# hongsukchoi/Pose2Mesh_RELEASE

Measured on NVIDIA H100. Metric: SMPL meshes/sec, higher is better.
Workload: dtype f32 (wgmma fp16x3 split, fp32 accumulate)

## Files before the change

pose2mesh_release_b200/csrc/cheb_umma.cu:

```cuda
#include <cuda.h>
#include <cuda_fp16.h>
#include <cuda_runtime.h>

#include <algorithm>
#include <climits>
#include <cstdlib>
#include <cstring>
#include <vector>

#include "p2m_internal.h"

namespace p2m {

namespace {

constexpr int TILE_M = 128;
constexpr int FC = 32;
constexpr int A_BLOCK_BYTES = TILE_M * 128;
constexpr float W_SCALE = 64.f;
constexpr float W_INV_SCALE = 1.f / 64.f;

struct TileHeader {
  int n_rows;
  int h1;
// ... 164 lines not shown
    fma4(acc0, __uint_as_float(a0.y), x0);
    fma4(acc1, __uint_as_float(a1.y), x1);
    fma4(acc0, __uint_as_float(a2.y), x2);
    fma4(acc1, __uint_as_float(a3.y), x3);
  }
  if (e + 1 < e1) {
    const uint2 a0 = lds_u2(ent + e * 8), a1 = lds_u2(ent + e * 8 + 8);
    const float4 x0 = lds_f4(rows_q + a0.x), x1 = lds_f4(rows_q + a1.x);
    fma4(acc0, __uint_as_float(a0.y), x0);
    fma4(acc1, __uint_as_float(a1.y), x1);
    e += 2;
  }
  if (e < e1) {
    const uint2 a0 = lds_u2(ent + e * 8);
    fma4(acc0, __uint_as_float(a0.y), lds_f4(rows_q + a0.x));
  }
  return make_float4(acc0.x + acc1.x, acc0.y + acc1.y, acc0.z + acc1.z, acc0.w + acc1.w);
}

__device__ __forceinline__ void wg_fence() { asm volatile("wgmma.fence.sync.aligned;" ::: "memory"); }
__device__ __forceinline__ void wg_commit() { asm volatile("wgmma.commit_group.sync.aligned;" ::: "memory"); }
__device__ __forceinline__ void wg_wait0() { asm volatile("wgmma.wait_group.sync.aligned 0;" ::: "memory"); }
template <int TA, int TB>
__device__ __forceinline__ void wgmma_m64n64(float (&d)[32], uint64_t desc_a, uint64_t desc_b) {
  asm volatile(
      "{\n\t.reg .pred p;\n\tsetp.ne.b32 p, 1, 0;\n\t"
      "wgmma.mma_async.sync.aligned.m64n64k16.f32.f16.f16 "
      "{%0, %1, %2, %3, %4, %5, %6, %7, %8, %9, %10, %11, %12, %13, %14, %15, "
      "%16, %17, %18, %19, %20, %21, %22, %23, %24, %25, %26, %27, %28, %29, %30, %31}, %32, %33, p, 1, 1, %34, %35;\n\t}"
      : "+f"(d[0]), "+f"(d[1]), "+f"(d[2]), "+f"(d[3]), "+f"(d[4]), "+f"(d[5]), "+f"(d[6]), "+f"(d[7]), "+f"(d[8]),
        "+f"(d[9]), "+f"(d[10]), "+f"(d[11]), "+f"(d[12]), "+f"(d[13]), "+f"(d[14]), "+f"(d[15]), "+f"(d[16]),
        "+f"(d[17]), "+f"(d[18]), "+f"(d[19]), "+f"(d[20]), "+f"(d[21]), "+f"(d[22]), "+f"(d[23]), "+f"(d[24]),
        "+f"(d[25]), "+f"(d[26]), "+f"(d[27]), "+f"(d[28]), "+f"(d[29]), "+f"(d[30]), "+f"(d[31])
      : "l"(desc_a), "l"(desc_b), "n"(TA), "n"(TB)
      : "memory");
}
template <int TA, int TB>
__device__ __forceinline__ void wgmma_m64n32(float (&d)[16], uint64_t desc_a, uint64_t desc_b) {
  asm volatile(
      "{\n\t.reg .pred p;\n\tsetp.ne.b32 p, 1, 0;\n\t"
      "wgmma.mma_async.sync.aligned.m64n32k16.f32.f16.f16 "
      "{%0, %1, %2, %3, %4, %5, %6, %7, %8, %9, %10, %11, %12, %13, %14, %15}, %16, %17, p, 1, 1, %18, %19;\n\t}"
      : "+f"(d[0]), "+f"(d[1]), "+f"(d[2]), "+f"(d[3]), "+f"(d[4]), "+f"(d[5]), "+f"(d[6]), "+f"(d[7]), "+f"(d[8]),
        "+f"(d[9]), "+f"(d[10]), "+f"(d[11]), "+f"(d[12]), "+f"(d[13]), "+f"(d[14]), "+f"(d[15])
      : "l"(desc_a), "l"(desc_b), "n"(TA), "n"(TB)
      : "memory");
}

__device__ __forceinline__ uint64_t make_desc_sw128(uint32_t saddr) {
  uint64_t d = 0;
  d |= (uint64_t)((saddr & 0x3FFFF) >> 4);
  d |= (uint64_t)1 << 16;
  d |= (uint64_t)(1024 >> 4) << 32;
  d |= (uint64_t)1 << 62;
  return d;
}

__host__ __device__ __forceinline__ uint32_t sw128_off(int row, int chunk) {
  return (uint32_t)row * 128u + (uint32_t)((chunk ^ (row & 7)) << 4);
}

struct Half4 {
  __half2 a, b;
};
__device__ __forceinline__ void split4(const float4& v, uint2& hi, uint2& lo) {
  __half2 h0 = __floats2half2_rn(v.x, v.y), h1 = __floats2half2_rn(v.z, v.w);
// ... 18 lines not shown
  EpiDev ep;
  int res_identity;
  const float* t1;
  const float* a_scale;
  const float* b_scale;
  long long ldy;
  int y_col0;
  float* y;
  int* status;
  long long* trace;
  int own_table;
  const float* head_wt;
  float* head_z;
  const unsigned char* apack;
  long long wslice_bytes;
  long long wblock_stride;
  int tma;
  CUtensorMap tm_x, tm_t1;
};

#ifdef P2M_UMMA_TRACE
__device__ __forceinline__ void trace_ev(const KParams& p, int role, int& n, int ev) {
  if (p.trace != nullptr && blockIdx.x == 0 && blockIdx.y == 0 && n < 512) {
    p.trace[role * 512 + n] = ((long long)ev << 48) | (clock64() & 0xFFFFFFFFFFFFll);
    ++n;
  }
}
#else
__device__ __forceinline__ void trace_ev(const KParams&, int, int&, int) {}
#endif

constexpr int W_PROD = 16;
constexpr int W_XLOAD = 16, N_XLOAD = 2, W_BLOAD = 18, W_EPI0 = 20;
constexpr int W_EPI1 = 8, W_PARK = 12;
constexpr int NUM_THREADS2 = 24 * 32;
constexpr int REGS_LAUNCH = 80, REGS_UTIL = 40, REGS_EPI = 120;
constexpr int REGS_PROD2 = 88, REGS_PARK = 24;
static_assert(128 * (REGS_EPI - REGS_LAUNCH) <= 128 * (REGS_LAUNCH - REGS_UTIL), "register pool balance");
static_assert(2 * 128 * (REGS_PROD2 - REGS_LAUNCH) + 2 * 128 * (REGS_EPI - REGS_LAUNCH) <=
                  128 * (REGS_LAUNCH - REGS_PARK) + 128 * (REGS_LAUNCH - REGS_UTIL),
              "register pool balance of the N = 128 layout");
static_assert(W_XLOAD % 4 == 0 && W_EPI0 % 4 == 0 && W_EPI0 - W_XLOAD == 4, "setmaxnreg works on aligned warpgroups");
static_assert(W_EPI1 % 4 == 0 && W_PARK == W_EPI1 + 4 && W_XLOAD == W_PARK + 4, "setmaxnreg works on aligned warpgroups");
template <int N>
__host__ __device__ constexpr int prod_warps() { return N == 128 ? W_EPI1 : W_PROD; }

template <int N>
__host__ __device__ constexpr int tile_rows() { return N == 128 ? 64 : TILE_M; }
template <int N, int NS, int XS, int MODE>
__global__ void __launch_bounds__(NUM_THREADS2, 1) k_cheb_conv_umma(const __grid_constant__ KParams p) {
  static_assert(N == 64 || N == 128, "one warpgroup holds the CTA's 128 x 64 or 64 x 128 accumulator in registers");
  constexpr int TM = tile_rows<N>();
  constexpr int NPW = prod_warps<N>();
  constexpr int NRG = NPW * 4;
  constexpr int RPT = TM / NRG;
  constexpr int NWG = N == 128 ? 2 : 1;
  static_assert(RPT == 2, "both configurations give a producer thread two tile rows");
  constexpr int H = TM / 64;
  constexpr int ER = 16 * H;
  constexpr bool KT1 = (MODE == 1);
  constexpr bool plain = !KT1;
  constexpr bool XDIRECT = KT1 && NS >= 3;
  constexpr int A_BYTES = TM * 128;
  constexpr int B_BLOCK_BYTES = N * 128;
  constexpr int SLOT_BYTES = A_BYTES + B_BLOCK_BYTES;

  extern __shared__ __align__(1024) unsigned char smem_raw[];
  unsigned char* ring = smem_raw;
  float* Xs = reinterpret_cast<float*>(ring + NS * SLOT_BYTES);
  const size_t xs_stage_floats = (XDIRECT && TM == 64) ? 0 : (size_t)TM * FC;
  float* T1s = Xs + XS * xs_stage_floats;
  const size_t t1_stage_floats = (size_t)p.max_h1 * FC;
  unsigned char* meta_s =
      reinterpret_cast<unsigned char*>(T1s + (plain ? 0 : XS) * t1_stage_floats);
  uint64_t* bars = reinterpret_cast<uint64_t*>(meta_s + 2 * (size_t)p.meta_stride);
  uint64_t* b_ab_full = bars;
  uint64_t* b_ab_empty = b_ab_full + NS;
  uint64_t* b_x_full = b_ab_empty + NS;
  uint64_t* b_x_empty = b_x_full + XS;
  uint64_t* b_m_full = b_x_empty + XS;
  uint64_t* b_m_empty = b_m_full + 2;
  uint64_t* b_stg_free = b_m_empty + 2;
  uint64_t* b_turn = b_stg_free + 1;
  uint32_t* flags = reinterpret_cast<uint32_t*>(b_turn + 1);
  volatile int* abort_flag = reinterpret_cast<volatile int*>(flags + 1);
  float* ep_mul = reinterpret_cast<float*>(flags + 4);
// ... 7 lines not shown
  uint64_t* b_res = reinterpret_cast<uint64_t*>(head_w_s);

  const int tid = threadIdx.x;
  const int warp = tid >> 5;
  const int lane = tid & 31;
  const int n_chunk = p.fin / FC;
  const int n_use = 3 * n_chunk;

  if (tid == 0) {
    for (int s = 0; s < NS; ++s) {
      mbar_init(smem_u32(b_ab_full + s), p.apack != nullptr ? 1 : NPW + 1);
      mbar_init(smem_u32(b_ab_empty + s), 4);
    }
    for (int s = 0; s < XS; ++s) {
      mbar_init(smem_u32(b_x_full + s), N_XLOAD * 32 + 1);
      mbar_init(smem_u32(b_x_empty + s), 1);
    }
    for (int s = 0; s < 2; ++s) {
      mbar_init(smem_u32(b_m_full + s), 1);
      mbar_init(smem_u32(b_m_empty + s), 1);
    }
    if (N == 128) {
      for (int w = 0; w < 4; ++w) mbar_init(smem_u32(b_res + w), 1);
      mbar_init(smem_u32(b_stg_free), 4);
      mbar_init(smem_u32(b_turn), 4);
    }
    *abort_flag = (smem_u32(ring) & 1023u) ? 1 : 0;
    if (*abort_flag) mbar_timeout(abort_flag, p.status, 100);
    fence_barrier_init();
  }
  const float a_scale = p.a_scale ? *p.a_scale : 1.f;
  const float b_inv = p.b_scale ? 1.f / *p.b_scale : W_INV_SCALE;
  const int ecol0 = (int)blockIdx.y * N;
  for (int n = threadIdx.x; n < N; n += NUM_THREADS2) {
    const float sc = (p.ep.scale ? p.ep.scale[ecol0 + n] : 1.f) / a_scale;
    const float sh = p.ep.scale ? p.ep.shift[ecol0 + n] : 0.f;
    const float bi = p.ep.bias ? p.ep.bias[ecol0 + n] : 0.f;
    ep_mul[n] = b_inv * sc;
    ep_add[n] = fmaf(bi, p.ep.scale ? p.ep.scale[ecol0 + n] : 1.f, sh);
  }
  if (N == 64 && p.head_z != nullptr)
    for (int i = threadIdx.x; i < 64 * 12; i += NUM_THREADS2) head_w_s[i] = p.head_wt[i];
  __syncthreads();

  const int mma_g = warp >= W_EPI0 ? 0 : (NWG == 2 && warp >= W_EPI1 && warp < W_PARK) ? 1 : -1;
  if (warp >= W_XLOAD && warp < W_EPI0) {
  asm volatile("setmaxnreg.dec.sync.aligned.u32 %0;" ::"n"(REGS_UTIL));
  if (warp >= W_XLOAD && warp < W_XLOAD + N_XLOAD) {
    if (p.apack == nullptr) {
      const int lt = tid - W_XLOAD * 32;
      const int lq = lt & 7, lrg = lt >> 3;
      const int my_tiles = (p.n_tiles - (int)blockIdx.x + (int)gridDim.x - 1) / (int)gridDim.x;
      if (lt == 32 && p.tma) {
        if (!XDIRECT) asm volatile("prefetch.tensormap [%0];" ::"l"(reinterpret_cast<uint64_t>(&p.tm_x)) : "memory");
        if (KT1) asm volatile("prefetch.tensormap [%0];" ::"l"(reinterpret_cast<uint64_t>(&p.tm_t1)) : "memory");
      }
      auto fetch_meta = [&](int itf) {
        const int pat = (blockIdx.x + itf * gridDim.x) % p.P;
        const int m = itf & 1;
        mbar_wait_relaxed(smem_u32(b_m_empty + m), ((itf >> 1) & 1) ^ 1, abort_flag, p.status, 1);
        const int mbytes = p.meta_bytes[pat];
        mbar_arrive_expect_tx(smem_u32(b_m_full + m), mbytes);
        bulk_g2s(smem_u32(meta_s + (size_t)m * p.meta_stride), p.meta + (size_t)pat * p.meta_stride, mbytes,
                 smem_u32(b_m_full + m));
      };
      if (lt == 0 && my_tiles > 0) fetch_meta(0);
      const uint32_t fin_bytes = (uint32_t)p.fin * 4u;
      const int sh = p.in_unpool ? 1 : 0;
      int g2 = 0;
      int ltn = 0;
      for (int it2 = 0; it2 < my_tiles; ++it2) {
        const int tile2 = blockIdx.x + it2 * gridDim.x;
        const long long mesh_row0 = (long long)(tile2 / p.P) * p.V;
        const int m2 = it2 & 1;
        mbar_wait_relaxed(smem_u32(b_m_full + m2), (it2 >> 1) & 1, abort_flag, p.status, 8);
        const unsigned char* mb2 = meta_s + (size_t)m2 * p.meta_stride;
        const TileHeader* hdr2 = reinterpret_cast<const TileHeader*>(mb2);
        const int* halo = reinterpret_cast<const int*>(mb2 + hdr2->off_halo);
        const int h1 = hdr2->h1;
        for (int c2 = 0; c2 < n_chunk; ++c2, ++g2) {
          const int xs2 = g2 % XS;
          mbar_wait_relaxed(smem_u32(b_x_empty + xs2), ((g2 / XS) & 1) ^ 1, abort_flag, p.status, 11);
          if (lt == 0) trace_ev(p, 4, ltn, 1);
// ... 8 lines not shown
                if (v[u] != -2) {
                  const uint32_t srow = (uint32_t)max(v[u], 0) >> shift;
                  cp_async16_zfill(dbase + (i0 + 8 * u) * 128, sbase + (uint64_t)srow * (uint64_t)fin_bytes,
                                   v[u] >= 0 ? 16u : 0u);
                }
              }
            }
          };
          const char* t1_mesh =
              reinterpret_cast<const char*>(KT1 ? p.t1 + mesh_row0 * p.fin + c2 * FC + lq * 4 : nullptr);
          const char* x_mesh = reinterpret_cast<const char*>(p.x + (mesh_row0 >> sh) * p.fin + c2 * FC + lq * 4);
          const uint32_t t1_dst = smem_u32(T1s + xs2 * t1_stage_floats) + lq * 16;
          const uint32_t x_dst = smem_u32(Xs + xs2 * xs_stage_floats) + lq * 16;
          if (p.tma) {
            if (lt == 32) {
              const int own0 = tile2 * TM;
              mbar_arrive_expect_tx(xbar, (XDIRECT ? 0 : (p.in_unpool ? TM / 2 : TM) * 128) + (KT1 ? TM * 128 : 0));
              if (!XDIRECT)
                tma_load_2d(smem_u32(Xs + xs2 * xs_stage_floats), &p.tm_x, c2 * FC, p.in_unpool ? own0 >> 1 : own0, xbar);
              if (KT1) tma_load_2d(smem_u32(T1s + xs2 * t1_stage_floats), &p.tm_t1, c2 * FC, own0, xbar);
            }
            if (KT1) stage_rows(t1_dst, t1_mesh, TM, h1, 0);
          } else {
            if (KT1) stage_rows(t1_dst, t1_mesh, 0, h1, 0);
            if (!XDIRECT) stage_rows(x_dst, x_mesh, 0, TM, sh);
            if (lt == 32) mbar_arrive(xbar);
          }
          cp_async_arrive_noinc(xbar);
          if (lt == 0) trace_ev(p, 4, ltn, 2);
          if (lt == 0 && c2 == (n_chunk > 1 ? 1 : 0) && it2 + 1 < my_tiles) fetch_meta(it2 + 1);
        }
      }
    }
  } else if (warp == W_BLOAD) {
    if (lane == 0) {
      uint32_t ucnt = 0;
      int tn = 0;
      const int uses = plain ? n_chunk : n_use;
      for (int tile = blockIdx.x; tile < p.n_tiles; tile += gridDim.x) {
        for (int u = 0; u < uses; ++u, ++ucnt) {
          const int s = ucnt % NS;
          const uint32_t par = (ucnt / NS) & 1;
          mbar_wait_relaxed(smem_u32(b_ab_empty + s), par ^ 1, abort_flag, p.status, 4);
          trace_ev(p, 1, tn, 10 + u);
          const unsigned char* wsl = p.wpack + (size_t)blockIdx.y * (size_t)p.wslice_bytes;
          if (p.apack != nullptr) {
            mbar_arrive_expect_tx(smem_u32(b_ab_full + s), B_BLOCK_BYTES + A_BYTES);
            bulk_g2s(smem_u32(ring + s * SLOT_BYTES), p.apack + ((size_t)tile * uses + u) * A_BYTES, A_BYTES,
                     smem_u32(b_ab_full + s));
          } else {
            mbar_arrive_expect_tx(smem_u32(b_ab_full + s), B_BLOCK_BYTES);
          }
          bulk_g2s(smem_u32(ring + s * SLOT_BYTES + A_BYTES), wsl + (size_t)u * (size_t)p.wblock_stride, B_BLOCK_BYTES,
                   smem_u32(b_ab_full + s));
        }
      }
    }
  }
  } else if (mma_g >= 0) {
    asm volatile("setmaxnreg.inc.sync.aligned.u32 %0;" ::"n"(REGS_EPI));
    const int g = mma_g;
    const int wq = warp - (g == 0 ? W_EPI0 : W_EPI1);
    const int tr = 3 + 2 * g;
    constexpr int CPR = EC / 4;
    constexpr int RPI = 32 / CPR;
    const uint32_t stg = smem_u32(epi_stage) + (uint32_t)wq * STG_WARP_BYTES;
    const int prow = lane / CPR, pc = lane % CPR;
    constexpr int NP = ER / RPI;
    int colk[2];
#pragma unroll
    for (int k = 0; k < 2; ++k) colk[k] = (int)(((uint32_t)pc ^ (uint32_t)((k * RPI + prow) & 7)) << 2);
    const int trow = (lane >> 4) * 64 + wq * 16 + (lane & 15);
    const int uses = plain ? n_chunk : n_use;
    int etn = 0;
    for (int it = g; (int)blockIdx.x + it * (int)gridDim.x < p.n_tiles; it += NWG) {
      const int tile = blockIdx.x + it * gridDim.x;
      const int b = tile / p.P, pat = tile - b * p.P;
      const long long mesh0 = (long long)b * p.V;
      int* own_w = own_s + (g * 4 + wq) * ER;
      {
        int v;
        if (lane >= ER) {
          v = -1;
        } else if (p.own_table) {
          v = __ldg(reinterpret_cast<const int*>(p.meta + (size_t)pat * p.meta_stride + 64) + trow);
        } else {
          v = pat * TM + trow;
          if (v >= p.V) v = -1;
        }
        __syncwarp();
        if (lane < ER) own_w[lane] = v;
        __syncwarp();
      }
      int own_v[NP];
#pragma unroll
      for (int i = 0; i < NP; ++i) own_v[i] = own_w[i * RPI + prow];
      if (p.ep.res != nullptr) {
        const bool own_cols = p.apack != nullptr || (N == 128 && p.res_identity);
        const int lpr = ((own_cols ? N : p.ep.res_F) * 4 + 127) >> 7;
        for (int j = lane; j < ER * lpr; j += 32) {
          const int rr = j / lpr, ln = j - rr * lpr;
          const int vtx = own_w[rr];
          if (vtx >= 0) {
            const long long r = mesh0 + vtx;
            prefetch_l2(p.ep.res + (p.ep.res_unpool ? (r >> 1) : r) * p.ep.res_F + (own_cols ? ecol0 : 0) + ln * 32);
          }
        }
      }
      float acc[2][32];
#pragma unroll
      for (int h = 0; h < 2; ++h)
#pragma unroll
        for (int j = 0; j < 32; ++j) acc[h][j] = 0.f;
      if (wq == 0 && lane == 0) trace_ev(p, tr, etn, 1);
      if (NWG == 2 && it > 0) {
        mbar_wait(smem_u32(b_turn), (uint32_t)(it - 1) & 1u, abort_flag, p.status, 13);
        if (wq == 0 && lane == 0) trace_ev(p, tr, etn, 3);
      }
      uint32_t ucnt = (uint32_t)it * (uint32_t)uses;
      for (int u = 0; u < uses; ++u, ++ucnt) {
        const uint32_t s = ucnt % NS;
        if (wq == 0 && lane == 0) trace_ev(p, tr, etn, 4);
        mbar_wait(smem_u32(b_ab_full + s), (ucnt / NS) & 1, abort_flag, p.status, 6);
        if (wq == 0 && lane == 0) trace_ev(p, tr, etn, 5);
        const uint32_t a0 = smem_u32(ring + s * SLOT_BYTES);
        wg_fence();
#pragma unroll
        for (int h = 0; h < 2; ++h) {
          const uint64_t da = make_desc_sw128(a0 + (TM == 128 ? (uint32_t)h * (64 * 128) : 0u));
          const uint64_t db = make_desc_sw128(a0 + A_BYTES + (TM == 64 ? (uint32_t)h * (64 * 128) : 0u));
          wgmma_m64n64<0, 0>(acc[h], da + 0, db + 0);
          wgmma_m64n64<0, 0>(acc[h], da + 2, db + 2);
          wgmma_m64n64<0, 0>(acc[h], da + 4, db + 0);
          wgmma_m64n64<0, 0>(acc[h], da + 6, db + 2);
          wgmma_m64n64<0, 0>(acc[h], da + 0, db + 4);
          wgmma_m64n64<0, 0>(acc[h], da + 2, db + 6);
        }
        wg_commit();
        wg_wait0();
        __syncwarp();
        if (lane == 0) mbar_arrive(smem_u32(b_ab_empty + s));
      }
      if (NWG == 2 && lane == 0) mbar_arrive(smem_u32(b_turn));
      if (wq == 0 && lane == 0) trace_ev(p, tr, etn, 2);
      auto stage_slab = [&](int cb) {
#pragma unroll
        for (int h = 0; h < H; ++h)
#pragma unroll
          for (int jj = 0; jj < 4; ++jj)
#pragma unroll
            for (int r = 0; r < 2; ++r) {
              const int lr = 16 * h + (lane >> 2) + 8 * r;
              const int cc = 8 * jj + 2 * (lane & 3);
              const int j = 4 * (cb / 8 + jj) + 2 * r;
              sts_f2(stg + lr * (EC * 4) + ((((uint32_t)(cc >> 2)) ^ (uint32_t)(lr & 7)) << 4) + (cc & 3) * 4,
                     acc[h][j], acc[h][j + 1]);
            }
        __syncwarp();
      };
      if (N == 64 && p.head_z != nullptr) {
        float z[12];
#pragma unroll
        for (int j = 0; j < 12; ++j) z[j] = 0.f;
#pragma unroll
        for (int cb = 0; cb < N; cb += 32) {
          stage_slab(cb);
#pragma unroll
          for (int c = 0; c < 8; ++c) {
            const float4 a = lds_f4(stg + lane * (EC * 4) + (((uint32_t)c ^ (uint32_t)(lane & 7)) << 4));
// ... 109 lines not shown
            const int n = cb + colk[i & 1];
            const int gn = ecol0 + n;
            const float4 a = lds_f4(stg + rr * (EC * 4) + (pc << 4));
            const int vtx = own_v[i];
            if (vtx >= 0) {
              const float4 mu = mu_k[i & 1], ad = ad_k[i & 1];
              float o[4] = {fmaf(a.x, mu.x, ad.x), fmaf(a.y, mu.y, ad.y), fmaf(a.z, mu.z, ad.z), fmaf(a.w, mu.w, ad.w)};
              if (p.ep.relu) {
#pragma unroll
                for (int e = 0; e < 4; ++e) o[e] = fmaxf(o[e], 0.f);
              }
              const long long r = mesh0 + vtx;
              if (p.ep.res != nullptr) {
                const float* res_row = p.ep.res + (p.ep.res_unpool ? (r >> 1) : r) * p.ep.res_F;
                if (p.res_identity) {
                  const float4 rv = __ldg(reinterpret_cast<const float4*>(res_row + gn));
                  o[0] += rv.x; o[1] += rv.y; o[2] += rv.z; o[3] += rv.w;
                } else {
#pragma unroll
                  for (int e = 0; e < 4; ++e) {
                    const float l = __ldg(p.ep.lam + gn + e);
                    o[e] += (1.f - l) * __ldg(res_row + __ldg(p.ep.i0 + gn + e)) + l * __ldg(res_row + __ldg(p.ep.i1 + gn + e));
                  }
                }
              }
              *reinterpret_cast<float4*>(p.y + r * p.ldy + p.y_col0 + gn) = make_float4(o[0], o[1], o[2], o[3]);
            }
          }
          __syncwarp();
        }
      }
    }
    if (N == 128 && lane < ER) bulk_wait0();
  } else if (warp >= NPW) {
    asm volatile("setmaxnreg.dec.sync.aligned.u32 %0;" ::"n"(REGS_PARK));
  } else {
    if (NPW != W_PROD) asm volatile("setmaxnreg.inc.sync.aligned.u32 %0;" ::"n"(REGS_PROD2));
    if (p.apack == nullptr) {
    const int q = tid & 7;
    const int rg = tid >> 3;
    const uint32_t t1s_a = smem_u32(T1s);
    const uint32_t ring_a = smem_u32(ring);
    const int my_tiles = (p.n_tiles - (int)blockIdx.x + (int)gridDim.x - 1) / (int)gridDim.x;
    const int n_stage = my_tiles * n_chunk;

    uint32_t row[RPT], re[RPT], ent_a = 0;
    int ptn = 0;
    uint32_t slot = 0, spar = 0;
    uint32_t so_f[RPT], so_s[RPT];
#pragma unroll
    for (int ps = 0; ps < RPT; ++ps) row[ps] = re[ps] = so_f[ps] = so_s[ps] = 0;
    const bool odd = (rg & 1) != 0;
    auto next_slot = [&]() {
      if (++slot == (uint32_t)NS) {
        slot = 0;
        spar ^= 1u;
      }
    };

    const int xsh = (p.tma && p.in_unpool) ? 1 : 0;
    const float* xp[RPT];
#pragma unroll
    for (int ps = 0; ps < RPT; ++ps) xp[ps] = nullptr;
    int it = 0, c = -1;
    for (int g = 0; g < n_stage; ++g) {
      if (++c == n_chunk) {
        c = 0;
        ++it;
      }
      const int m = it & 1;
// ... 107 lines not shown
#pragma unroll
        for (int ps = 0; ps < RPT; ++ps) t1v[ps] = lds_f4(t1s_q + row[ps] * 128);
        if (tid == 0) trace_ev(p, 0, ptn, 6);
        {
          uint32_t s2 = slot + 2, p2 = spar;
          if (s2 >= (uint32_t)NS) {
            s2 -= (uint32_t)NS;
            p2 ^= 1u;
          }
          mbar_wait(smem_u32(b_ab_empty + s2), p2 ^ 1u, abort_flag, p.status, 10);
        }
        emit(x);
        emit(t1v);
#pragma unroll
        for (int ps = 0; ps < RPT; ++ps) t2[ps] = cheb_t2(t2[ps], x[ps]);
        emit(t2);
      }
      if (NS >= 3) {
        fence_async_proxy();
        __syncwarp();
        if ((tid & 31) == 0) {
#pragma unroll
          for (int k = 0; k < 3; ++k) mbar_arrive(smem_u32(b_ab_full + (slot0 + k) % NS));
        }
      }
      if (tid == 0) trace_ev(p, 0, ptn, 7);
      producer_barrier<NPW * 32>();
      if (tid == 0) trace_ev(p, 0, ptn, 8);
      if (tid == 0) mbar_arrive(smem_u32(b_x_empty + xs));
      if (tid == 0 && c == n_chunk - 1) mbar_arrive(smem_u32(b_m_empty + m));
    }
    }
  }
}

struct DwParams {
  const float* x;
  int in_unpool;
  int V, P, fin;
  int n_tiles;
  const unsigned char* meta;
  const int* meta_bytes;
  int meta_stride, max_h1;
  const float* g;
  int fout_total, m_off, m_cols;
  int chunk0;
  const float* a_scale;
  float* dw;
  int* status;
  const float* t1;
  int g_unpool;
  int swap;
  int tma;
  CUtensorMap tm_x, tm_t1;
};

__device__ __forceinline__ uint64_t make_desc_sw128_mn(uint32_t saddr, uint32_t lbo_bytes) {
  uint64_t d = 0;
  d |= (uint64_t)((saddr & 0x3FFFF) >> 4);
  d |= (uint64_t)((lbo_bytes >> 4) & 0x3FFF) << 16;
  d |= (uint64_t)(1024 >> 4) << 32;
  d |= (uint64_t)1 << 62;
  return d;
}

constexpr int DW_NS = 3;
// ... 439 lines not shown
  for (int ns = N == WIDE_N ? 6 : 3; ns >= 3; ns -= 3)
    for (int xs = 2; xs >= 1; --xs)
      if (smem_bytes_for(N, ns, xs, t, t1_given) <= SMEM_LIMIT) return {ns, xs};
  return {0, 0};
}

typedef CUresult (*TmapEncodeFn)(CUtensorMap*, CUtensorMapDataType, cuuint32_t, void*, const cuuint64_t*, const cuuint64_t*,
                                 const cuuint32_t*, const cuuint32_t*, CUtensorMapInterleave, CUtensorMapSwizzle,
                                 CUtensorMapL2promotion, CUtensorMapFloatOOBfill);
TmapEncodeFn tmap_encoder() {
  static TmapEncodeFn fn = [] {
    void* f = nullptr;
    cudaDriverEntryPointQueryResult q;
    if (cudaGetDriverEntryPoint("cuTensorMapEncodeTiled", &f, cudaEnableDefault, &q) != cudaSuccess ||
        q != cudaDriverEntryPointSuccess)
      f = nullptr;
    return reinterpret_cast<TmapEncodeFn>(f);
  }();
  return fn;
}
bool make_row_tmap(CUtensorMap* tm, const float* base, long long rows, int fin, int box_rows) {
  TmapEncodeFn enc = tmap_encoder();
  if (enc == nullptr || (reinterpret_cast<uintptr_t>(base) & 15u) != 0) return false;
  const cuuint64_t dims[2] = {(cuuint64_t)fin, (cuuint64_t)rows};
  const cuuint64_t strides[1] = {(cuuint64_t)fin * 4};
  const cuuint32_t box[2] = {(cuuint32_t)FC, (cuuint32_t)box_rows};
  const cuuint32_t estr[2] = {1, 1};
  return enc(tm, CU_TENSOR_MAP_DATA_TYPE_FLOAT32, 2, const_cast<float*>(base), dims, strides, box, estr,
             CU_TENSOR_MAP_INTERLEAVE_NONE, CU_TENSOR_MAP_SWIZZLE_NONE, CU_TENSOR_MAP_L2_PROMOTION_L2_128B,
             CU_TENSOR_MAP_FLOAT_OOB_FILL_NONE) == CUDA_SUCCESS;
}

template <int N, int NS, int XS, int MODE>
int check_launch_regs() {
  static int state = 0;
  if (state == 0) {
    cudaFuncAttributes fa;
    P2M_CUDA_OK(cudaFuncGetAttributes(&fa, k_cheb_conv_umma<N, NS, XS, MODE>));
    state = (fa.numRegs == REGS_LAUNCH) ? 1 : -1;
  }
  if (state < 0) {
    set_error("k_cheb_conv_umma was compiled with a register count other than the one its setmaxnreg split assumes");
    return P2M_ERR_CUDA;
  }
  return P2M_OK;
}

template <int N, int NS, int XS>
int launch_cfg(const UmmaConvArgs& a, int* status, const float* zero_row, int sm_count, cudaStream_t s) {
  constexpr int TM = tile_rows<N>();
  const DevLevel& g = *a.g;
  const TileBlobs& t = conv_tiles(N, g, a.tiles);
  const size_t smem = smem_bytes_for(N, NS, XS, t, !a.plain);
  auto kern = a.plain ? k_cheb_conv_umma<N, NS, XS, 0> : k_cheb_conv_umma<N, NS, XS, 1>;
  P2M_CUDA_OK(cudaFuncSetAttribute(kern, cudaFuncAttributeMaxDynamicSharedMemorySize, (int)smem));
  P2M_TRY((a.plain ? check_launch_regs<N, NS, XS, 0>() : check_launch_regs<N, NS, XS, 1>()));
  KParams p;
  p.x = a.x;
  p.in_unpool = a.in_unpool;
  p.V = g.V;
  p.P = t.n_pattern;
  p.fin = a.fin;
  p.meta = t.meta;
  p.meta_bytes = t.bytes;
  p.meta_stride = t.stride;
  p.max_h1 = t.max_h1;
  p.own_table = a.tiles != nullptr ? 1 : 0;
  p.n_tiles = a.batch * p.P;
  p.wpack = static_cast<const unsigned char*>(a.wpack);
  p.apack = nullptr;
  p.wslice_bytes = (long long)N * 128;
  p.wblock_stride = (long long)a.fout * 128;
  p.zero_row = zero_row;
  p.ep = to_dev(a.ep);
  p.res_identity = (a.ep.res != nullptr && a.ep.res_F == a.fout) ? 1 : 0;
  p.y = a.y;
  p.t1 = a.t1;
  p.a_scale = a.a_scale;
  p.b_scale = nullptr;
  p.ldy = a.ldy > 0 ? a.ldy : a.fout;
  p.y_col0 = a.y_col0;
  p.status = status;
  p.trace = a.trace;
  p.head_wt = a.fout == 64 ? a.head_wt : nullptr;
  p.head_z = a.fout == 64 ? a.head_z : nullptr;
  if (N == WIDE_N) {
    const bool y_ok = (reinterpret_cast<uintptr_t>(p.y) & 15u) == 0 && (p.ldy * 4) % 16 == 0 && (p.y_col0 * 4) % 16 == 0;
    const bool res_ok = !p.res_identity || ((reinterpret_cast<uintptr_t>(p.ep.res) & 15u) == 0 && (p.ep.res_F * 4) % 16 == 0);
    if (!y_ok || !res_ok) {
      set_error("umma_conv: the 128-column epilogue needs 16-byte aligned output and identity-residual rows");
      return P2M_ERR_INVALID;
    }
  }
  p.tma = 0;
  std::memset(&p.tm_x, 0, sizeof(p.tm_x));
  std::memset(&p.tm_t1, 0, sizeof(p.tm_t1));
  if (a.tiles == nullptr && g.V % TILE_M == 0 && g_umma_tma) {
    const long long rows = (long long)a.batch * g.V;
    bool ok = make_row_tmap(&p.tm_x, a.x, a.in_unpool ? rows / 2 : rows, a.fin, a.in_unpool ? TM / 2 : TM);
    if (ok && a.t1 != nullptr) ok = make_row_tmap(&p.tm_t1, a.t1, rows, a.fin, TM);
    p.tma = ok ? 1 : 0;
  }
  const int n_slices = a.fout / N;
  const dim3 grid(std::min(p.n_tiles, std::max(1, sm_count / n_slices)), n_slices);
  kern<<<grid, NUM_THREADS2, smem, s>>>(p);
  P2M_LAUNCH_OK();
  return P2M_OK;
}

int launch_n(const UmmaConvArgs& a, int* status, const float* zero_row, int sm_count, cudaStream_t s) {
  const int N = conv_n(a.fout);
  const ConvCfg c = conv_cfg(N, conv_tiles(N, *a.g, a.tiles), !a.plain);
  if (c.ns == 0) {
    set_error("umma_conv: tile family does not fit shared memory");
    return P2M_ERR_INVALID;
  }
  if (N == CONV_N)
    return c.xs == 2 ? launch_cfg<CONV_N, 3, 2>(a, status, zero_row, sm_count, s)
                     : launch_cfg<CONV_N, 3, 1>(a, status, zero_row, sm_count, s);
  if (c.ns == 6)
    return c.xs == 2 ? launch_cfg<WIDE_N, 6, 2>(a, status, zero_row, sm_count, s)
                     : launch_cfg<WIDE_N, 6, 1>(a, status, zero_row, sm_count, s);
  return c.xs == 2 ? launch_cfg<WIDE_N, 3, 2>(a, status, zero_row, sm_count, s)
                   : launch_cfg<WIDE_N, 3, 1>(a, status, zero_row, sm_count, s);
}

}

namespace {
void balance_store_halves(std::vector<unsigned short>* ord) {
  std::vector<unsigned short> q0, q1;
  for (unsigned short r : *ord) ((r & 4) ? q1 : q0).push_back(r);
  if (q0.size() != q1.size() || (q0.size() & 1)) return;
  size_t o = 0;
  for (size_t g = 0; g + 1 < q0.size(); g += 2) {
    (*ord)[o++] = q0[g];
    (*ord)[o++] = q0[g + 1];
    (*ord)[o++] = q1[g];
// ... 241 lines not shown
  kern<<<batch * t.n_pattern, 512, smem, s>>>(p);
  P2M_LAUNCH_OK();
  return P2M_OK;
}

bool umma_conv_supported(const DevLevel& g, int fin, int fout) {
  if (g.meta128.n_pattern <= 0) return false;
  if (fin % FC != 0 || fin < FC || fin > 256) return false;
  if (g.meta128.max_h1 > 256) return false;
  if (fout != 64 && fout != 128 && fout != 256) return false;
  const int N = conv_n(fout);
  const TileBlobs& t = conv_tiles(N, g, nullptr);
  return t.n_pattern > 0 && smem_bytes_for(N, 3, 1, t, true) <= SMEM_LIMIT && smem_bytes_for(N, 3, 1, t, false) <= SMEM_LIMIT;
}

int umma_conv_x_stages(const DevLevel& g, int fout, bool plain) {
  const int N = conv_n(fout);
  return conv_cfg(N, conv_tiles(N, g, nullptr), !plain).xs;
}
bool umma_tma_rows(const DevLevel& g) { return g.V % TILE_M == 0 && g_umma_tma && tmap_encoder() != nullptr; }

size_t umma_plain_pack_bytes(int N, int K) { return (size_t)(K / FC) * N * 128; }

static size_t gemm_x_image_bytes(int M, int K) { return (size_t)((M + TILE_M - 1) / TILE_M) * (K / FC) * A_BLOCK_BYTES; }
size_t umma_gemm_apack_bytes(int M, int K) { return gemm_x_image_bytes(M, K) + 128; }
size_t umma_gemm_wpack_bytes(int N, int K) { return (size_t)(K / FC) * N * 128; }
bool umma_gemm_supported(int M, int N, int K) { return M > 0 && K >= FC && K % FC == 0 && N >= 64 && N % 64 == 0; }

namespace {
template <int N>
int launch_gemm_cfg(KParams p, int n_slices, int sm_count, cudaStream_t s) {
  constexpr int NS = 3;
  const size_t smem = smem_bytes_for(N, NS, 1, TileBlobs(), false);
  auto kern = k_cheb_conv_umma<N, NS, 1, 0>;
  P2M_TRY((check_launch_regs<N, NS, 1, 0>()));
  P2M_CUDA_OK(cudaFuncSetAttribute(kern, cudaFuncAttributeMaxDynamicSharedMemorySize, (int)smem));
  p.wslice_bytes = (long long)umma_gemm_wpack_bytes(N, p.fin);
  p.wblock_stride = (long long)N * 128;
  const dim3 grid(std::min(p.n_tiles, sm_count), n_slices);
  kern<<<grid, NUM_THREADS2, smem, s>>>(p);
  P2M_LAUNCH_OK();
  return P2M_OK;
}
}

int launch_umma_gemm(GemmOperand X, GemmOperand W, int M, int N, int K, const Epilogue& ep, float* Y, void* apack,
                     void* wpack, int* status, int sm_count, cudaStream_t s, int n_real, int k_real,
                     const float* x_scale, const float* w_scale) {
  if (n_real <= 0 || n_real > N) n_real = N;
  if (k_real <= 0 || k_real > K) k_real = K;
  if (!umma_gemm_supported(M, N, K) || (ep.res != nullptr && ep.res_F != N)) {
    set_error("umma_gemm: unsupported shape");
    return P2M_ERR_INVALID;
  }
  const int tiles = (M + TILE_M - 1) / TILE_M;
  const int ns = CONV_N;
  if (x_scale == nullptr) {
    float* sc = reinterpret_cast<float*>(static_cast<unsigned char*>(apack) + gemm_x_image_bytes(M, K));
    P2M_TRY(launch_absmax_scale(X.p, (M - 1) * X.ld_row + (k_real - 1) * X.ld_k + 1, sc, s));
    x_scale = sc;
  }
  P2M_TRY(launch_pack(PackSrc{X.p, X.ld_row, X.ld_k, TILE_M, K / FC, 1, M, 1.f, 0, 0.f, k_real, x_scale},
                      (long long)tiles * (K / FC), apack, s));
  P2M_TRY(launch_pack(PackSrc{W.p, W.ld_row, W.ld_k, ns, K / FC, 1, n_real, w_scale ? 1.f : W_SCALE, 0, 0.f, k_real,
                              w_scale},
                      (long long)(N / ns) * (K / FC), wpack, s));
  KParams p;
  std::memset(&p, 0, sizeof(p));
  p.V = M;
  p.P = tiles;
  p.fin = K;
  p.n_tiles = tiles;
  p.wpack = static_cast<const unsigned char*>(wpack);
// ... 46 lines not shown
```

Measured before the change: 12030.

## Split wide N=128 conv into its own 640-thread kernel using m64n128 wgmma

```diff
diff --git a/pose2mesh_release_b200/csrc/cheb_umma.cu b/pose2mesh_release_b200/csrc/cheb_umma.cu
--- a/pose2mesh_release_b200/csrc/cheb_umma.cu
+++ b/pose2mesh_release_b200/csrc/cheb_umma.cu
@@ -220,6 +220,28 @@
         "+f"(d[9]), "+f"(d[10]), "+f"(d[11]), "+f"(d[12]), "+f"(d[13]), "+f"(d[14]), "+f"(d[15]), "+f"(d[16]),
         "+f"(d[17]), "+f"(d[18]), "+f"(d[19]), "+f"(d[20]), "+f"(d[21]), "+f"(d[22]), "+f"(d[23]), "+f"(d[24]),
         "+f"(d[25]), "+f"(d[26]), "+f"(d[27]), "+f"(d[28]), "+f"(d[29]), "+f"(d[30]), "+f"(d[31])
+      : "l"(desc_a), "l"(desc_b), "n"(TA), "n"(TB)
+      : "memory");
+}
+template <int TA, int TB>
+__device__ __forceinline__ void wgmma_m64n128(float (&d)[2][32], uint64_t desc_a, uint64_t desc_b) {
+  asm volatile(
+      "{\n\t.reg .pred p;\n\tsetp.ne.b32 p, 1, 0;\n\t"
+      "wgmma.mma_async.sync.aligned.m64n128k16.f32.f16.f16 "
+      "{%0, %1, %2, %3, %4, %5, %6, %7, %8, %9, %10, %11, %12, %13, %14, %15, "
+      "%16, %17, %18, %19, %20, %21, %22, %23, %24, %25, %26, %27, %28, %29, %30, %31, "
+      "%32, %33, %34, %35, %36, %37, %38, %39, %40, %41, %42, %43, %44, %45, %46, %47, "
+      "%48, %49, %50, %51, %52, %53, %54, %55, %56, %57, %58, %59, %60, %61, %62, %63}, %64, %65, p, 1, 1, %66, %67;\n\t}"
+      : "+f"(d[0][0]), "+f"(d[0][1]), "+f"(d[0][2]), "+f"(d[0][3]), "+f"(d[0][4]), "+f"(d[0][5]), "+f"(d[0][6]),
+        "+f"(d[0][7]), "+f"(d[0][8]), "+f"(d[0][9]), "+f"(d[0][10]), "+f"(d[0][11]), "+f"(d[0][12]), "+f"(d[0][13]),
+        "+f"(d[0][14]), "+f"(d[0][15]), "+f"(d[0][16]), "+f"(d[0][17]), "+f"(d[0][18]), "+f"(d[0][19]), "+f"(d[0][20]),
+        "+f"(d[0][21]), "+f"(d[0][22]), "+f"(d[0][23]), "+f"(d[0][24]), "+f"(d[0][25]), "+f"(d[0][26]), "+f"(d[0][27]),
+        "+f"(d[0][28]), "+f"(d[0][29]), "+f"(d[0][30]), "+f"(d[0][31]), "+f"(d[1][0]), "+f"(d[1][1]), "+f"(d[1][2]),
+        "+f"(d[1][3]), "+f"(d[1][4]), "+f"(d[1][5]), "+f"(d[1][6]), "+f"(d[1][7]), "+f"(d[1][8]), "+f"(d[1][9]),
+        "+f"(d[1][10]), "+f"(d[1][11]), "+f"(d[1][12]), "+f"(d[1][13]), "+f"(d[1][14]), "+f"(d[1][15]), "+f"(d[1][16]),
+        "+f"(d[1][17]), "+f"(d[1][18]), "+f"(d[1][19]), "+f"(d[1][20]), "+f"(d[1][21]), "+f"(d[1][22]), "+f"(d[1][23]),
+        "+f"(d[1][24]), "+f"(d[1][25]), "+f"(d[1][26]), "+f"(d[1][27]), "+f"(d[1][28]), "+f"(d[1][29]), "+f"(d[1][30]),
+        "+f"(d[1][31])
       : "l"(desc_a), "l"(desc_b), "n"(TA), "n"(TB)
       : "memory");
 }
@@ -304,26 +326,43 @@
 
 constexpr int W_PROD = 16;
 constexpr int W_XLOAD = 16, N_XLOAD = 2, W_BLOAD = 18, W_EPI0 = 20;
-constexpr int W_EPI1 = 8, W_PARK = 12;
 constexpr int NUM_THREADS2 = 24 * 32;
 constexpr int REGS_LAUNCH = 80, REGS_UTIL = 40, REGS_EPI = 120;
-constexpr int REGS_PROD2 = 88, REGS_PARK = 24;
 static_assert(128 * (REGS_EPI - REGS_LAUNCH) <= 128 * (REGS_LAUNCH - REGS_UTIL), "register pool balance");
-static_assert(2 * 128 * (REGS_PROD2 - REGS_LAUNCH) + 2 * 128 * (REGS_EPI - REGS_LAUNCH) <=
-                  128 * (REGS_LAUNCH - REGS_PARK) + 128 * (REGS_LAUNCH - REGS_UTIL),
-              "register pool balance of the N = 128 layout");
 static_assert(W_XLOAD % 4 == 0 && W_EPI0 % 4 == 0 && W_EPI0 - W_XLOAD == 4, "setmaxnreg works on aligned warpgroups");
-static_assert(W_EPI1 % 4 == 0 && W_PARK == W_EPI1 + 4 && W_XLOAD == W_PARK + 4, "setmaxnreg works on aligned warpgroups");
+constexpr int W_PROD_W = 8, W_EPI1_W = 8, W_XLOAD_W = 12, W_BLOAD_W = 14, W_EPI0_W = 16;
+constexpr int NUM_THREADS_W = 20 * 32;
+constexpr int REGS_LAUNCH_W = 96, REGS_UTIL_W = 40, REGS_PROD_W = 88, REGS_EPI_W = 128;
+static_assert(2 * 128 * (REGS_EPI_W - REGS_LAUNCH_W) <=
+                  128 * (REGS_LAUNCH_W - REGS_UTIL_W) + 2 * 128 * (REGS_LAUNCH_W - REGS_PROD_W),
+              "register pool balance of the 64 x 128 layout");
+static_assert(REGS_LAUNCH_W * NUM_THREADS_W <= 65536 && (REGS_LAUNCH_W + 8) * NUM_THREADS_W > 65536,
+              "__launch_bounds__(NUM_THREADS_W, 1) gives REGS_LAUNCH_W registers per thread");
+static_assert(W_EPI1_W == W_PROD_W && W_EPI1_W % 4 == 0 && W_XLOAD_W == W_EPI1_W + 4 && W_EPI0_W == W_XLOAD_W + 4 &&
+                  (W_EPI0_W + 4) * 32 == NUM_THREADS_W,
+              "setmaxnreg works on aligned warpgroups");
 template <int N>
-__host__ __device__ constexpr int prod_warps() { return N == 128 ? W_EPI1 : W_PROD; }
+struct ConvRoles {
+  static constexpr int threads = NUM_THREADS2, prod = W_PROD, xload = W_XLOAD, bload = W_BLOAD, epi0 = W_EPI0,
+                       epi1 = -1;
+  static constexpr int regs_launch = REGS_LAUNCH, regs_util = REGS_UTIL, regs_prod = REGS_LAUNCH, regs_epi = REGS_EPI;
+};
+template <>
+struct ConvRoles<128> {
+  static constexpr int threads = NUM_THREADS_W, prod = W_PROD_W, xload = W_XLOAD_W, bload = W_BLOAD_W,
+                       epi0 = W_EPI0_W, epi1 = W_EPI1_W;
+  static constexpr int regs_launch = REGS_LAUNCH_W, regs_util = REGS_UTIL_W, regs_prod = REGS_PROD_W,
+                       regs_epi = REGS_EPI_W;
+};
 
 template <int N>
 __host__ __device__ constexpr int tile_rows() { return N == 128 ? 64 : TILE_M; }
 template <int N, int NS, int XS, int MODE>
-__global__ void __launch_bounds__(NUM_THREADS2, 1) k_cheb_conv_umma(const __grid_constant__ KParams p) {
+__device__ __forceinline__ void cheb_conv_body(const KParams& p) {
   static_assert(N == 64 || N == 128, "one warpgroup holds the CTA's 128 x 64 or 64 x 128 accumulator in registers");
+  using R = ConvRoles<N>;
   constexpr int TM = tile_rows<N>();
-  constexpr int NPW = prod_warps<N>();
+  constexpr int NPW = R::prod;
   constexpr int NRG = NPW * 4;
   constexpr int RPT = TM / NRG;
   constexpr int NWG = N == 128 ? 2 : 1;
@@ -397,7 +436,7 @@
   const float a_scale = p.a_scale ? *p.a_scale : 1.f;
   const float b_inv = p.b_scale ? 1.f / *p.b_scale : W_INV_SCALE;
   const int ecol0 = (int)blockIdx.y * N;
-  for (int n = threadIdx.x; n < N; n += NUM_THREADS2) {
+  for (int n = threadIdx.x; n < N; n += R::threads) {
     const float sc = (p.ep.scale ? p.ep.scale[ecol0 + n] : 1.f) / a_scale;
     const float sh = p.ep.scale ? p.ep.shift[ecol0 + n] : 0.f;
     const float bi = p.ep.bias ? p.ep.bias[ecol0 + n] : 0.f;
@@ -405,15 +444,15 @@
     ep_add[n] = fmaf(bi, p.ep.scale ? p.ep.scale[ecol0 + n] : 1.f, sh);
   }
   if (N == 64 && p.head_z != nullptr)
-    for (int i = threadIdx.x; i < 64 * 12; i += NUM_THREADS2) head_w_s[i] = p.head_wt[i];
+    for (int i = threadIdx.x; i < 64 * 12; i += R::threads) head_w_s[i] = p.head_wt[i];
   __syncthreads();
 
-  const int mma_g = warp >= W_EPI0 ? 0 : (NWG == 2 && warp >= W_EPI1 && warp < W_PARK) ? 1 : -1;
-  if (warp >= W_XLOAD && warp < W_EPI0) {
-  asm volatile("setmaxnreg.dec.sync.aligned.u32 %0;" ::"n"(REGS_UTIL));
-  if (warp >= W_XLOAD && warp < W_XLOAD + N_XLOAD) {
+  const int mma_g = warp >= R::epi0 ? 0 : (NWG == 2 && warp >= R::epi1 && warp < R::epi1 + 4) ? 1 : -1;
+  if (warp >= R::xload && warp < R::epi0) {
+  asm volatile("setmaxnreg.dec.sync.aligned.u32 %0;" ::"n"(R::regs_util));
+  if (warp >= R::xload && warp < R::xload + N_XLOAD) {
     if (p.apack == nullptr) {
-      const int lt = tid - W_XLOAD * 32;
+      const int lt = tid - R::xload * 32;
       const int lq = lt & 7, lrg = lt >> 3;
       const int my_tiles = (p.n_tiles - (int)blockIdx.x + (int)gridDim.x - 1) / (int)gridDim.x;
       if (lt == 32 && p.tma) {
@@ -488,7 +527,7 @@
         }
       }
     }
-  } else if (warp == W_BLOAD) {
+  } else if (warp == R::bload) {
     if (lane == 0) {
       uint32_t ucnt = 0;
       int tn = 0;
@@ -514,9 +553,9 @@
     }
   }
   } else if (mma_g >= 0) {
-    asm volatile("setmaxnreg.inc.sync.aligned.u32 %0;" ::"n"(REGS_EPI));
+    asm volatile("setmaxnreg.inc.sync.aligned.u32 %0;" ::"n"(R::regs_epi));
     const int g = mma_g;
-    const int wq = warp - (g == 0 ? W_EPI0 : W_EPI1);
+    const int wq = warp - (g == 0 ? R::epi0 : R::epi1);
     const int tr = 3 + 2 * g;
     constexpr int CPR = EC / 4;
     constexpr int RPI = 32 / CPR;
@@ -581,16 +620,27 @@
         if (wq == 0 && lane == 0) trace_ev(p, tr, etn, 5);
         const uint32_t a0 = smem_u32(ring + s * SLOT_BYTES);
         wg_fence();
-#pragma unroll
-        for (int h = 0; h < 2; ++h) {
-          const uint64_t da = make_desc_sw128(a0 + (TM == 128 ? (uint32_t)h * (64 * 128) : 0u));
-          const uint64_t db = make_desc_sw128(a0 + A_BYTES + (TM == 64 ? (uint32_t)h * (64 * 128) : 0u));
-          wgmma_m64n64<0, 0>(acc[h], da + 0, db + 0);
-          wgmma_m64n64<0, 0>(acc[h], da + 2, db + 2);
-          wgmma_m64n64<0, 0>(acc[h], da + 4, db + 0);
-          wgmma_m64n64<0, 0>(acc[h], da + 6, db + 2);
-          wgmma_m64n64<0, 0>(acc[h], da + 0, db + 4);
-          wgmma_m64n64<0, 0>(acc[h], da + 2, db + 6);
+        if constexpr (N == 128) {
+          const uint64_t da = make_desc_sw128(a0);
+          const uint64_t db = make_desc_sw128(a0 + A_BYTES);
+          wgmma_m64n128<0, 0>(acc, da + 0, db + 0);
+          wgmma_m64n128<0, 0>(acc, da + 2, db + 2);
+          wgmma_m64n128<0, 0>(acc, da + 4, db + 0);
+          wgmma_m64n128<0, 0>(acc, da + 6, db + 2);
+          wgmma_m64n128<0, 0>(acc, da + 0, db + 4);
+          wgmma_m64n128<0, 0>(acc, da + 2, db + 6);
+        } else {
+#pragma unroll
+          for (int h = 0; h < 2; ++h) {
+            const uint64_t da = make_desc_sw128(a0 + (uint32_t)h * (64 * 128));
+            const uint64_t db = make_desc_sw128(a0 + A_BYTES);
+            wgmma_m64n64<0, 0>(acc[h], da + 0, db + 0);
+            wgmma_m64n64<0, 0>(acc[h], da + 2, db + 2);
+            wgmma_m64n64<0, 0>(acc[h], da + 4, db + 0);
+            wgmma_m64n64<0, 0>(acc[h], da + 6, db + 2);
+            wgmma_m64n64<0, 0>(acc[h], da + 0, db + 4);
+            wgmma_m64n64<0, 0>(acc[h], da + 2, db + 6);
+          }
         }
         wg_commit();
         wg_wait0();
@@ -766,10 +816,8 @@
       }
     }
     if (N == 128 && lane < ER) bulk_wait0();
-  } else if (warp >= NPW) {
-    asm volatile("setmaxnreg.dec.sync.aligned.u32 %0;" ::"n"(REGS_PARK));
   } else {
-    if (NPW != W_PROD) asm volatile("setmaxnreg.inc.sync.aligned.u32 %0;" ::"n"(REGS_PROD2));
+    if (R::regs_prod < R::regs_launch) asm volatile("setmaxnreg.dec.sync.aligned.u32 %0;" ::"n"(R::regs_prod));
     if (p.apack == nullptr) {
     const int q = tid & 7;
     const int rg = tid >> 3;
@@ -943,6 +991,16 @@
     }
     }
   }
+}
+
+template <int N, int NS, int XS, int MODE>
+__global__ void __launch_bounds__(NUM_THREADS2, 1) k_cheb_conv_umma(const __grid_constant__ KParams p) {
+  static_assert(N == 64, "the 64 x 128 configuration is k_cheb_conv_wide");
+  cheb_conv_body<N, NS, XS, MODE>(p);
+}
+template <int NS, int XS, int MODE>
+__global__ void __launch_bounds__(NUM_THREADS_W, 1) k_cheb_conv_wide(const __grid_constant__ KParams p) {
+  cheb_conv_body<128, NS, XS, MODE>(p);
 }
 
 struct DwParams {
@@ -1448,15 +1506,22 @@
 }
 
 template <int N, int NS, int XS, int MODE>
+constexpr auto conv_kernel() {
+  if constexpr (N == WIDE_N) return k_cheb_conv_wide<NS, XS, MODE>;
+  else return k_cheb_conv_umma<N, NS, XS, MODE>;
+}
+template <int N, int NS, int XS, int MODE>
 int check_launch_regs() {
   static int state = 0;
   if (state == 0) {
     cudaFuncAttributes fa;
-    P2M_CUDA_OK(cudaFuncGetAttributes(&fa, k_cheb_conv_umma<N, NS, XS, MODE>));
-    state = (fa.numRegs == REGS_LAUNCH) ? 1 : -1;
+    P2M_CUDA_OK(cudaFuncGetAttributes(&fa, conv_kernel<N, NS, XS, MODE>()));
+    state = (fa.numRegs == ConvRoles<N>::regs_launch) ? 1 : -1;
   }
   if (state < 0) {
-    set_error("k_cheb_conv_umma was compiled with a register count other than the one its setmaxnreg split assumes");
+    set_error(N == WIDE_N
+                  ? "k_cheb_conv_wide was compiled with a register count other than the one its setmaxnreg split assumes"
+                  : "k_cheb_conv_umma was compiled with a register count other than the one its setmaxnreg split assumes");
     return P2M_ERR_CUDA;
   }
   return P2M_OK;
@@ -1468,7 +1533,7 @@
   const DevLevel& g = *a.g;
   const TileBlobs& t = conv_tiles(N, g, a.tiles);
   const size_t smem = smem_bytes_for(N, NS, XS, t, !a.plain);
-  auto kern = a.plain ? k_cheb_conv_umma<N, NS, XS, 0> : k_cheb_conv_umma<N, NS, XS, 1>;
+  auto kern = a.plain ? conv_kernel<N, NS, XS, 0>() : conv_kernel<N, NS, XS, 1>();
   P2M_CUDA_OK(cudaFuncSetAttribute(kern, cudaFuncAttributeMaxDynamicSharedMemorySize, (int)smem));
   P2M_TRY((a.plain ? check_launch_regs<N, NS, XS, 0>() : check_launch_regs<N, NS, XS, 1>()));
   KParams p;
@@ -1519,7 +1584,7 @@
   }
   const int n_slices = a.fout / N;
   const dim3 grid(std::min(p.n_tiles, std::max(1, sm_count / n_slices)), n_slices);
-  kern<<<grid, NUM_THREADS2, smem, s>>>(p);
+  kern<<<grid, ConvRoles<N>::threads, smem, s>>>(p);
   P2M_LAUNCH_OK();
   return P2M_OK;
 }
@@ -1827,13 +1892,13 @@
 int launch_gemm_cfg(KParams p, int n_slices, int sm_count, cudaStream_t s) {
   constexpr int NS = 3;
   const size_t smem = smem_bytes_for(N, NS, 1, TileBlobs(), false);
-  auto kern = k_cheb_conv_umma<N, NS, 1, 0>;
+  auto kern = conv_kernel<N, NS, 1, 0>();
   P2M_TRY((check_launch_regs<N, NS, 1, 0>()));
   P2M_CUDA_OK(cudaFuncSetAttribute(kern, cudaFuncAttributeMaxDynamicSharedMemorySize, (int)smem));
   p.wslice_bytes = (long long)umma_gemm_wpack_bytes(N, p.fin);
   p.wblock_stride = (long long)N * 128;
   const dim3 grid(std::min(p.n_tiles, sm_count), n_slices);
-  kern<<<grid, NUM_THREADS2, smem, s>>>(p);
+  kern<<<grid, ConvRoles<N>::threads, smem, s>>>(p);
   P2M_LAUNCH_OK();
   return P2M_OK;
 }
```

After: 12420, median of 6. 1.03x the previous value.
